# preethamam/AutomaticPanoramicImageStitching-AutoPanoStitch-MATLAB

Hardware: AMD Instinct MI355X
Metric: MPix/s end-to-end stitch (SIFT->blend), 64x4K images (higher is better)
Workload: dtype f32; 1 GPU

## Files before the change

### automaticpanoramicimagestitching-autopanostitch-matlab_amd/csrc/sift.hip

```cpp
#include <algorithm>
#include <cmath>
#include <cstring>
#include <vector>
#ifdef APS_DBG
#include <atomic>
#include <map>
#include <mutex>
#endif

#include "aps_internal.h"

#include <rocprim/rocprim.hpp>

namespace aps {

constexpr int kBorder = 5;
constexpr int kMaxInterp = 5;
constexpr int kOriBins = 36;
constexpr float kFix = 1048576.0f;

__device__ __forceinline__ long long to_fix(float v) { return (long long)(int)rintf(v * kFix); }
constexpr float kFltEps = 1.1920928955078125e-07f;

__device__ __forceinline__ float poly_exp2(float f) {
// ... 773 lines not shown
                                   unsigned int* __restrict__ flag) {
    const unsigned int i = blockIdx.x * blockDim.x + threadIdx.x;
    if (i >= n) return;
    flag[i] = (i == 0 || keys[i] != keys[i - 1]) ? 1u : 0u;
}
__global__ void compact_recs_kernel(const KpRec* __restrict__ recs, const unsigned int* __restrict__ idx,
                                    const unsigned int* __restrict__ flag, const unsigned int* __restrict__ pos,
                                    unsigned int n, KpRec* __restrict__ out) {
    const unsigned int i = blockIdx.x * blockDim.x + threadIdx.x;
    if (i >= n || !flag[i]) return;
    out[pos[i]] = recs[idx[i]];
}

struct PyrTable {
    OctaveDesc oct[16];
    int n_oct, nl;
    float sigma;
};

constexpr int kMW = 256;
constexpr int kMI = kMW - 8;
struct ExtremaPlan {
    int blk_ptr[17];
    int nstrip[16];
    int ch[16];
};

template <int nl>
__global__ __launch_bounds__(256) void extrema_march_kernel(const PyrTable* __restrict__ pt, ExtremaPlan plan, float thr,
                                                            unsigned long long* __restrict__ cells,
                                                            unsigned int* __restrict__ count, unsigned int cap) {
    constexpr int NG = nl + 3, ND = nl + 2, RING = 6, TW = kMW;
    __shared__ __attribute__((aligned(16))) float s_d[ND][RING * TW];
    constexpr int kLocalCap = 256;
    __shared__ unsigned long long s_cells[kLocalCap];
    __shared__ unsigned int s_n, s_base;
    int o = 0;
    while (o < 15 && (int)blockIdx.x >= plan.blk_ptr[o + 1]) ++o;
    const OctaveDesc& od = pt->oct[o];
    const int w = od.w, h = od.h;
    const int local = (int)blockIdx.x - plan.blk_ptr[o];
    const int strip = local % plan.nstrip[o], chunk = local / plan.nstrip[o];
    const int x0 = strip * kMI - 4, y0 = chunk * plan.ch[o], y1 = min(y0 + plan.ch[o], h);
    const int tid = threadIdx.x;
    if (tid == 0) s_n = 0u;
    const __attribute__((address_space(1))) float* G[NG];
#pragma unroll
    for (int p = 0; p < NG; ++p) G[p] = (const __attribute__((address_space(1))) float*)od.G[p];
    const int lx4 = tid & 63, lr = tid >> 6;
    const int gx = x0 + 4 * lx4;
    const bool vec = (w & 3) == 0 && gx >= 0 && gx + 3 < w;
    auto fetch = [&](int row, float4 g[NG]) __attribute__((always_inline)) {
        const size_t rowoff = (size_t)min(max(row, 0), h - 1) * w;
        if (vec) {
#pragma unroll
            for (int p = 0; p < NG; ++p) {
                typedef float f32x4g __attribute__((ext_vector_type(4)));
                const f32x4g v = *reinterpret_cast<const __attribute__((address_space(1))) f32x4g*>(G[p] + rowoff + gx);
                g[p] = make_float4(v.x, v.y, v.z, v.w);
            }
        } else {
            const size_t o0 = rowoff + min(max(gx, 0), w - 1), o1 = rowoff + min(max(gx + 1, 0), w - 1);
            const size_t o2 = rowoff + min(max(gx + 2, 0), w - 1), o3 = rowoff + min(max(gx + 3, 0), w - 1);
#pragma unroll
            for (int p = 0; p < NG; ++p) g[p] = make_float4(G[p][o0], G[p][o1], G[p][o2], G[p][o3]);
        }
    };
    auto park = [&](int row, const float4 g[NG]) __attribute__((always_inline)) {
        const int slot = (row - (y0 - 1)) % RING;
#pragma unroll
        for (int p = 0; p < ND; ++p)
            *reinterpret_cast<float4*>(&s_d[p][slot * TW + 4 * lx4]) =
                make_float4(g[p + 1].x - g[p].x, g[p + 1].y - g[p].y, g[p + 1].z - g[p].z, g[p + 1].w - g[p].w);
    };
    float4 g[NG];
    if (lr < 2) {
        fetch(y0 - 1 + lr, g);
        park(y0 - 1 + lr, g);
    }
    fetch(y0 + 1 + lr, g);
    const int lx = tid, c = x0 + lx;
    const int lxc = min(max(lx, 1), kMW - 2);
    const bool col_ok = lx >= 4 && lx < kMW - 4 && c >= kBorder && c < w - kBorder;
    for (int ys = y0; ys < y1; ys += 4) {
        park(ys + 1 + lr, g);
        if (ys + 4 < y1) fetch(ys + 5 + lr, g);
        __syncthreads();
        const int base = (ys - y0) % RING;
        float wmax[3][4], wmin[3][4];
#pragma unroll
        for (int p = 0; p < ND; ++p) {
            float hmx[6], hmn[6];
#pragma unroll
            for (int rr = 0; rr < 6; ++rr) {
                int slot = base + rr;
                slot = slot >= RING ? slot - RING : slot;
                const float* row = &s_d[p][slot * TW + lxc - 1];
                hmx[rr] = fmaxf(fmaxf(row[0], row[1]), row[2]);
                hmn[rr] = fminf(fminf(row[0], row[1]), row[2]);
            }
#pragma unroll
            for (int k = 0; k < 4; ++k) {
                wmax[p % 3][k] = fmaxf(fmaxf(hmx[k], hmx[k + 1]), hmx[k + 2]);
                wmin[p % 3][k] = fminf(fminf(hmn[k], hmn[k + 1]), hmn[k + 2]);
            }
            if (p < 2) continue;
            const int layer = p - 1;
#pragma unroll
            for (int k = 0; k < 4; ++k) {
                const int r = ys + k;
                if (!col_ok || r >= y1 || r < kBorder || r >= h - kBorder) continue;
                int slot = base + k + 1;
                slot = slot >= RING ? slot - RING : slot;
                const float val = s_d[layer][slot * TW + lx];
                if (!(fabsf(val) > thr)) continue;
                const float mx = fmaxf(fmaxf(wmax[0][k], wmax[1][k]), wmax[2][k]);
                const float mn = fminf(fminf(wmin[0][k], wmin[1][k]), wmin[2][k]);
                const bool is_max = val > 0 && val >= mx, is_min = val < 0 && val <= mn;
                if (!(is_max || is_min)) continue;
                const unsigned long long cell = ((unsigned long long)o << 40) | ((unsigned long long)layer << 32) |
                                                ((unsigned long long)r << 16) | (unsigned long long)c;
                const unsigned int loc = atomicAdd(&s_n, 1u);
                if (loc < (unsigned)kLocalCap) {
                    s_cells[loc] = cell;
                } else {
                    const unsigned int slot2 = atomicAdd(count, 1u);
                    if (slot2 < cap) cells[slot2] = cell;
                }
            }
        }
        __syncthreads();
    }
    const unsigned int n_loc = min(s_n, (unsigned)kLocalCap);
    if (n_loc == 0u) return;
    if (tid == 0) s_base = atomicAdd(count, n_loc);
    __syncthreads();
    for (unsigned int e = tid; e < n_loc; e += 256) {
        const unsigned int slot = s_base + e;
        if (slot < cap) cells[slot] = s_cells[e];
    }
}

constexpr int kWS = 124;
constexpr int kWCells = 256;
struct ExtremaWavePlan {
    int job_ptr[17];
    int nstrip[16];
    int ch[16];
};

__device__ __forceinline__ float dpp_from_lower_lane(float v) {
    return __int_as_float(__builtin_amdgcn_update_dpp(__float_as_int(v), __float_as_int(v), 0x138, 0xf, 0xf, false));
}
__device__ __forceinline__ float dpp_from_upper_lane(float v) {
    return __int_as_float(__builtin_amdgcn_update_dpp(__float_as_int(v), __float_as_int(v), 0x130, 0xf, 0xf, false));
}

template <int nl>
__global__ __launch_bounds__(256) void extrema_wave_kernel(const PyrTable* __restrict__ pt, ExtremaWavePlan plan, float thr,
                                                           unsigned long long* __restrict__ cells,
                                                           unsigned int* __restrict__ count, unsigned int cap) {
    constexpr int NG = nl + 3, ND = nl + 2;
    __shared__ unsigned long long s_cells[4][kWCells];
    const int lane = threadIdx.x & 63;
    const int wave = __builtin_amdgcn_readfirstlane(threadIdx.x >> 6);
    const int job = (int)blockIdx.x * 4 + wave;
    if (job >= plan.job_ptr[16]) return;
    int o = 0;
    while (o < 15 && job >= plan.job_ptr[o + 1]) ++o;
    const OctaveDesc& od = pt->oct[o];
    const int w = od.w, h = od.h;
    const int local = job - plan.job_ptr[o];
    const int strip = local % plan.nstrip[o], chunk = local / plan.nstrip[o];
    const int x0 = strip * kWS - 2, y0 = chunk * plan.ch[o], y1 = min(y0 + plan.ch[o], h);
    const int rc0 = max(y0, kBorder), rc1 = min(y1, h - kBorder);
    if (rc0 >= rc1) return;
    const __attribute__((address_space(1))) float* G[NG];
#pragma unroll
    for (int p = 0; p < NG; ++p) G[p] = (const __attribute__((address_space(1))) float*)od.G[p];
    const int c0 = x0 + 2 * lane;
    const int cb = min(max(c0, 0), w - 2);
    const bool own = lane >= 1 && lane <= 62;
    const bool ok0 = own && c0 >= kBorder && c0 < w - kBorder, ok1 = own && c0 + 1 >= kBorder && c0 + 1 < w - kBorder;
    typedef float f32x2g __attribute__((ext_vector_type(2)));
    f32x2g q[3][NG];
    auto fetch = [&](auto S, int row) __attribute__((always_inline)) {
        constexpr int sl = decltype(S)::value;
        const size_t off = (size_t)min(row, h - 1) * w + cb;
#pragma unroll
        for (int p = 0; p < NG; ++p) q[sl][p] = *reinterpret_cast<const __attribute__((address_space(1))) f32x2g*>(G[p] + off);
    };
    float hm[3][ND][2], hn[3][ND][2];
    float dc[3][nl][2];
    auto reduce_row = [&](auto S) __attribute__((always_inline)) {
        constexpr int sl = decltype(S)::value;
#pragma unroll
        for (int p = 0; p < ND; ++p) {
            const float d0 = q[sl][p + 1].x - q[sl][p].x, d1 = q[sl][p + 1].y - q[sl][p].y;
            const float lf = dpp_from_lower_lane(d1), rt = dpp_from_upper_lane(d0);
            hm[sl][p][0] = fmaxf(fmaxf(lf, d0), d1);
            hm[sl][p][1] = fmaxf(fmaxf(d0, d1), rt);
            hn[sl][p][0] = fminf(fminf(lf, d0), d1);
            hn[sl][p][1] = fminf(fminf(d0, d1), rt);
            if (p >= 1 && p <= nl) {
                dc[sl][p - 1][0] = d0;
                dc[sl][p - 1][1] = d1;
            }
        }
    };
    int qn = 0;
    auto emit = [&](bool pass, int layer, int r, int c) __attribute__((always_inline)) {
        const unsigned long long m = __ballot(pass);
        if (m == 0ull) return;
        if (pass) {
            const unsigned long long cell = ((unsigned long long)o << 40) | ((unsigned long long)layer << 32) |
                                            ((unsigned long long)r << 16) | (unsigned long long)c;
            const int at = qn + __popcll(m & ((1ull << lane) - 1ull));
            if (at < kWCells) {
                s_cells[wave][at] = cell;
            } else {
                const unsigned int slot2 = atomicAdd(count, 1u);
                if (slot2 < cap) cells[slot2] = cell;
            }
        }
        qn += __popcll(m);
    };
    auto test_row = [&](auto SA, auto SB, auto SC, int r) __attribute__((always_inline)) {
        constexpr int a = decltype(SA)::value, b = decltype(SB)::value, c = decltype(SC)::value;
        float wmax[3][2], wmin[3][2];
#pragma unroll
        for (int p = 0; p < ND; ++p) {
#pragma unroll
            for (int k = 0; k < 2; ++k) {
                wmax[p % 3][k] = fmaxf(fmaxf(hm[a][p][k], hm[b][p][k]), hm[c][p][k]);
                wmin[p % 3][k] = fminf(fminf(hn[a][p][k], hn[b][p][k]), hn[c][p][k]);
            }
            if (p < 2) continue;
            const int layer = p - 1;
#pragma unroll
            for (int k = 0; k < 2; ++k) {
                const float val = dc[b][layer - 1][k];
                const float mx = fmaxf(fmaxf(wmax[0][k], wmax[1][k]), wmax[2][k]);
                const float mn = fminf(fminf(wmin[0][k], wmin[1][k]), wmin[2][k]);
                const bool pass = (k ? ok1 : ok0) && fabsf(val) > thr && ((val > 0 && val >= mx) || (val < 0 && val <= mn));
                emit(pass, layer, r, c0 + k);
            }
        }
    };
    using I0 = std::integral_constant<int, 0>;
    using I1 = std::integral_constant<int, 1>;
    using I2 = std::integral_constant<int, 2>;
    fetch(I0{}, rc0 - 1);
    fetch(I1{}, rc0);
    fetch(I2{}, rc0 + 1);
    reduce_row(I0{});
    fetch(I0{}, rc0 + 2);
    reduce_row(I1{});
    fetch(I1{}, rc0 + 3);
    for (int r = rc0; r < rc1; r += 3) {
        reduce_row(I2{});
        fetch(I2{}, r + 4);
        test_row(I0{}, I1{}, I2{}, r);
        if (r + 1 >= rc1) break;
        reduce_row(I0{});
        fetch(I0{}, r + 5);
        test_row(I1{}, I2{}, I0{}, r + 1);
        if (r + 2 >= rc1) break;
        reduce_row(I1{});
        fetch(I1{}, r + 6);
        test_row(I2{}, I0{}, I1{}, r + 2);
    }
    if (qn == 0) return;
    const int n_loc = min(qn, kWCells);
    unsigned int base = 0;
    if (lane == 0) base = atomicAdd(count, (unsigned int)n_loc);
    base = __builtin_amdgcn_readfirstlane(base);
    __builtin_amdgcn_wave_barrier();
    for (int e = lane; e < n_loc; e += 64) {
        const unsigned int slot = base + e;
        if (slot < cap) cells[slot] = s_cells[wave][e];
    }
}

__global__ void refine_kernel(const PyrTable* __restrict__ pt, const unsigned long long* __restrict__ cells,
                              const unsigned int* __restrict__ n_cells, unsigned int cells_cap, float contr_thr,
                              float edge_thr, KpRec* __restrict__ recs, unsigned int* __restrict__ count,
                              unsigned int cap) {
    const unsigned int i = blockIdx.x * blockDim.x + threadIdx.x;
    const unsigned int n = min(*n_cells, cells_cap);
    if (i >= n) return;
    const unsigned long long key = cells[i];
    const int o = (int)(key >> 40), layer = (int)((key >> 32) & 0xff), r = (int)((key >> 16) & 0xffff),
              c = (int)(key & 0xffff);
    KpRec kp;
    if (!adjust_extremum(pt->oct[o], pt->nl, o, layer, r, c, contr_thr, edge_thr, kp)) return;
    const unsigned int slot = atomicAdd(count, 1u);
    if (slot < cap) recs[slot] = kp;
}

__device__ __forceinline__ float kp_scale(float sigma, int layer, float xi, int nl) {
    return sigma * my_exp2(((float)layer + xi) / (float)nl);
}

__global__ __launch_bounds__(256) void orient_kernel(const PyrTable* __restrict__ pt,
                                                     const KpRec* __restrict__ kps, unsigned int n,
                                                     unsigned int* __restrict__ ori_count,
                                                     float* __restrict__ ori_angle ,
                                                     unsigned char* __restrict__ ori_bin ) {
    __shared__ unsigned long long s_hist[4][kOriBins];
    __shared__ float s_h[4][kOriBins + 4];
    const int wv = threadIdx.x >> 6, lane = threadIdx.x & 63;
    const unsigned int ki = blockIdx.x * 4 + wv;
    const bool active = ki < n;
    if (lane < kOriBins) s_hist[wv][lane] = 0ull;
    __syncthreads();
    int o = 0, layer = 1, r0 = 0, c0 = 0;
    float xi = 0;
    if (active) {
        const KpRec kp = kps[ki];
        o = (int)(kp.key >> 40);
        layer = (int)((kp.key >> 32) & 0xff);
        r0 = (int)((kp.key >> 16) & 0xffff);
        c0 = (int)(kp.key & 0xffff);
        xi = kp.xi;
    }
    const OctaveDesc& od = pt->oct[o];
    const __attribute__((address_space(1))) float* g = (const __attribute__((address_space(1))) float*)od.G[layer];
    const int w = od.w, h = od.h;
    const float scl = kp_scale(pt->sigma, layer, xi, pt->nl);
    const int radius = (int)rintf(4.5f * scl);
    const float sig = 1.5f * scl;
    const float expf_scale = -1.0f / (2.0f * sig * sig);
    const int side = 2 * radius + 1;
    if (active) {
        for (int s = lane; s < side * side; s += 64) {
            const int i = s / side - radius, j = s % side - radius;
            const int y = r0 + i, x = c0 + j;
            if (y <= 0 || y >= h - 1 || x <= 0 || x >= w - 1) continue;
            const int ctr = y * w + x;
            const float dx = g[ctr + 1] - g[ctr - 1];
            const float dy = g[ctr - w] - g[ctr + w];
            const float wgt = my_exp((float)(i * i + j * j) * expf_scale);
            const float ori = fast_atan2_deg(dy, dx);
            const float mag = sqrtf(dx * dx + dy * dy);
            int bin = (int)rintf(((float)kOriBins / 360.0f) * ori);
            if (bin >= kOriBins) bin -= kOriBins;
            if (bin < 0) bin += kOriBins;
            const long long q = to_fix(wgt * mag);
            atomicAdd(&s_hist[wv][bin], (unsigned long long)q);
        }
    }
    __syncthreads();
    if (lane < kOriBins) s_h[wv][lane + 2] = (float)(long long)s_hist[wv][lane] * (1.0f / kFix);
    __syncthreads();
    if (lane < 2) {
        s_h[wv][lane] = s_h[wv][kOriBins + lane];
        s_h[wv][kOriBins + 2 + lane] = s_h[wv][2 + lane];
    }
    __syncthreads();
    float hv = 0.f;
    if (lane < kOriBins)
        hv = (s_h[wv][lane] + s_h[wv][lane + 4]) * (1.0f / 16.0f) + (s_h[wv][lane + 1] + s_h[wv][lane + 3]) * (4.0f / 16.0f) +
             s_h[wv][lane + 2] * (6.0f / 16.0f);
    __syncthreads();
    if (lane < kOriBins) s_h[wv][lane] = hv;
    __syncthreads();
    if (active) {
        float omax = lane < kOriBins ? s_h[wv][lane] : -INFINITY;
#pragma unroll
        for (int off = 32; off > 0; off >>= 1) omax = fmaxf(omax, __shfl_xor(omax, off));
        const float thr = omax * 0.8f;
        bool peak = false;
        float angle = 0.f;
        if (lane < kOriBins) {
            const int j = lane;
            const int l = j > 0 ? j - 1 : kOriBins - 1, r2 = j < kOriBins - 1 ? j + 1 : 0;
            const float hj = s_h[wv][j], hl = s_h[wv][l], hr = s_h[wv][r2];
            if (hj > hl && hj > hr && hj >= thr) {
                peak = true;
                float bin = (float)j + 0.5f * (hl - hr) / (hl - 2.0f * hj + hr);
                bin = bin < 0 ? (float)kOriBins + bin : (bin >= (float)kOriBins ? bin - (float)kOriBins : bin);
                angle = 360.0f - (360.0f / (float)kOriBins) * bin;
                if (fabsf(angle - 360.0f) < kFltEps) angle = 0.0f;
            }
        }
        const unsigned long long pm = __ballot(peak);
        if (peak) {
            const unsigned int cnt = (unsigned int)__popcll(pm & ((1ull << lane) - 1ull));
            ori_angle[(size_t)ki * kOriBins + cnt] = angle;
            ori_bin[(size_t)ki * kOriBins + cnt] = (unsigned char)lane;
        }
        if (lane == 0) ori_count[ki] = (unsigned int)__popcll(pm);
    }
}

struct OrientedKp {
    unsigned int kp;
    float angle;
};

__global__ void expand_oriented_kernel(const unsigned int* __restrict__ ori_count,
                                       const unsigned int* __restrict__ ori_pos,
                                       const float* __restrict__ ori_angle, unsigned int n,
                                       OrientedKp* __restrict__ out) {
    const unsigned int i = blockIdx.x * blockDim.x + threadIdx.x;
    if (i >= n) return;
    const unsigned int c = ori_count[i], p = ori_pos[i];
    for (unsigned int e = 0; e < c; ++e) {
        out[p + e].kp = i;
        out[p + e].angle = ori_angle[(size_t)i * kOriBins + e];
    }
}

constexpr int kD = 4, kN = 8, kHistLen = (kD + 2) * (kD + 2) * (kN + 2);
constexpr int kDescQueue = 512;

__global__ __launch_bounds__(256) void descr_kernel(const PyrTable* __restrict__ pt,
                                                    const KpRec* __restrict__ kps,
                                                    const OrientedKp* __restrict__ oks, unsigned int n_out,
                                                    float* __restrict__ desc, int desc_layout, int64_t ldd,
                                                    double* __restrict__ loc, int64_t ldl,
                                                    float* __restrict__ aux, int plain_sweep) {
    __shared__ unsigned long long s_hist[4][kHistLen];
    __shared__ __attribute__((aligned(16))) float s_raw[4][128];
    __shared__ int s_queue[4][kDescQueue];
    const int wv = threadIdx.x >> 6, lane = threadIdx.x & 63;
    const unsigned int oi = blockIdx.x * 4 + wv;
    const bool active = oi < n_out;
    for (int e = lane; e < kHistLen; e += 64) s_hist[wv][e] = 0ull;
    __syncthreads();
    int o = 0, layer = 1, r0 = 0, c0 = 0;
    float xc = 0, xr = 0, xi = 0, contr = 0, kangle = 0;
    if (active) {
        const OrientedKp ok = oks[oi];
        const KpRec kp = kps[ok.kp];
        o = (int)(kp.key >> 40);
        layer = (int)((kp.key >> 32) & 0xff);
        r0 = (int)((kp.key >> 16) & 0xffff);
        c0 = (int)(kp.key & 0xffff);
        xc = kp.xc;
        xr = kp.xr;
        xi = kp.xi;
        contr = kp.contr;
        kangle = ok.angle;
    }
    const OctaveDesc& od = pt->oct[o];
    const __attribute__((address_space(1))) float* g = (const __attribute__((address_space(1))) float*)od.G[layer];
    const int w = od.w, h = od.h;
    const float scl = kp_scale(pt->sigma, layer, xi, pt->nl);
    float ori = 360.0f - kangle;
    if (fabsf(ori - 360.0f) < kFltEps) ori = 0.0f;
    const float ptx = (float)c0 + xc, pty = (float)r0 + xr;
    const int px = (int)rintf(ptx), py = (int)rintf(pty);
    float sin_t, cos_t;
    sincos_deg(ori, sin_t, cos_t);
    const float bins_per_deg = (float)kN / 360.0f;
    const float exp_scale = -1.0f / ((float)(kD * kD) * 0.5f);
    const float hist_width = 3.0f * scl;
    int radius = (int)rintf(hist_width * 1.4142135623730951f * (float)(kD + 1) * 0.5f);
    const int diag = (int)sqrt((double)w * w + (double)h * h);
    if (radius > diag) radius = diag;
    cos_t = cos_t / hist_width;
    sin_t = sin_t / hist_width;
    const int side = 2 * radius + 1;
    (void)side;
    auto accumulate = [&](int i, int j) __attribute__((always_inline)) {
        const float c_rot = (float)j * cos_t - (float)i * sin_t;
        const float r_rot = (float)j * sin_t + (float)i * cos_t;
        float rbin = r_rot + (float)(kD / 2) - 0.5f;
        float cbin = c_rot + (float)(kD / 2) - 0.5f;
        const int r = py + i, c = px + j;
        const int ctr = r * w + c;
        const float dx = g[ctr + 1] - g[ctr - 1];
        const float dy = g[ctr - w] - g[ctr + w];
        const float wgt = my_exp((c_rot * c_rot + r_rot * r_rot) * exp_scale);
        const float o_deg = fast_atan2_deg(dy, dx);
        const float mag = sqrtf(dx * dx + dy * dy) * wgt;
        float obin = (o_deg - ori) * bins_per_deg;
        const int rr0 = (int)floorf(rbin), cc0 = (int)floorf(cbin);
        int o0 = (int)floorf(obin);
        rbin -= (float)rr0;
        cbin -= (float)cc0;
        obin -= (float)o0;
        if (o0 < 0) o0 += kN;
        if (o0 >= kN) o0 -= kN;
        const float v_r1 = mag * rbin, v_r0 = mag - v_r1;
        const float v_rc11 = v_r1 * cbin, v_rc10 = v_r1 - v_rc11;
        const float v_rc01 = v_r0 * cbin, v_rc00 = v_r0 - v_rc01;
        const float v111 = v_rc11 * obin, v110 = v_rc11 - v111;
        const float v101 = v_rc10 * obin, v100 = v_rc10 - v101;
        const float v011 = v_rc01 * obin, v010 = v_rc01 - v011;
        const float v001 = v_rc00 * obin, v000 = v_rc00 - v001;
        const int idx = ((rr0 + 1) * (kD + 2) + cc0 + 1) * (kN + 2) + o0;
        unsigned long long* hb = &s_hist[wv][idx];
#define ADDQ(off, v) atomicAdd(hb + (off), (unsigned long long)to_fix(v))
        ADDQ(0, v000);
        ADDQ(1, v001);
        ADDQ(kN + 2, v010);
        ADDQ(kN + 3, v011);
        ADDQ((kD + 2) * (kN + 2), v100);
        ADDQ((kD + 2) * (kN + 2) + 1, v101);
        ADDQ((kD + 3) * (kN + 2), v110);
        ADDQ((kD + 3) * (kN + 2) + 1, v111);
#undef ADDQ
    };
    if (active) {
        int* q = s_queue[wv];
        int qn = 0;
        auto flush = [&]() __attribute__((always_inline)) {
            const int rounds = (qn + 63) >> 6;
            __builtin_amdgcn_wave_barrier();
            const int e0 = lane * rounds;
            int pk = q[min(e0, kDescQueue - 1)];
            for (int r = 0; r < rounds; ++r) {
                const int e = e0 + r;
                const int pk_next = q[min(e + 1, kDescQueue - 1)];
                if (e < qn) accumulate(pk >> 16, (int)(short)(pk & 0xffff));
                pk = pk_next;
            }
            __builtin_amdgcn_wave_barrier();
            qn = 0;
        };
        auto passes = [&](int i, int j) __attribute__((always_inline)) {
            const float c_rot = (float)j * cos_t - (float)i * sin_t;
            const float r_rot = (float)j * sin_t + (float)i * cos_t;
            const float rbin = r_rot + (float)(kD / 2) - 0.5f;
            const float cbin = c_rot + (float)(kD / 2) - 0.5f;
            const int r = py + i, c = px + j;
            return j >= -radius && j <= radius && rbin > -1 && rbin < kD && cbin > -1 && cbin < kD && r > 0 && r < h - 1 && c > 0 && c < w - 1;
        };
        bool plain = plain_sweep != 0 || radius > 63 || fabsf(sin_t) < 1e-4f || fabsf(cos_t) < 1e-4f;
        int jl_[2] = {0, 0}, len_[2] = {0, 0};
        if (!plain) {
            bool bad = false;
#pragma unroll
            for (int half = 0; half < 2; ++half) {
                const int i = -radius + lane + 64 * half;
                const bool row_ok = i <= radius && py + i > 0 && py + i < h - 1;
                const float fi = (float)i;
                float lo = fmaxf(-(float)radius, (float)(1 - px)), hi = fminf((float)radius, (float)(w - 2 - px));
                auto clip = [&](float a, float lo_v, float hi_v) __attribute__((always_inline)) {
                    const float p0 = lo_v / a, p1 = hi_v / a;
                    lo = fmaxf(lo, fminf(p0, p1));
                    hi = fminf(hi, fmaxf(p0, p1));
                };
                clip(sin_t, -2.5f - fi * cos_t, 2.5f - fi * cos_t);
                clip(cos_t, -2.5f + fi * sin_t, 2.5f + fi * sin_t);
                const int gl = (int)ceilf(lo), gh = (int)floorf(hi);
                int jl = 0x7fffffff, jh = -0x7fffffff;
#pragma unroll
                for (int dlt = 2; dlt >= -2; --dlt)
                    if (passes(i, gl + dlt)) jl = gl + dlt;
#pragma unroll
                for (int dlt = -2; dlt <= 2; ++dlt)
                    if (passes(i, gh + dlt)) jh = gh + dlt;
                const bool none = jl > jh;
                bool good;
                if (none)
                    good = gl > gh;
                else
                    good = !passes(i, jl - 1) && !passes(i, jh + 1) && passes(i, (jl + jh) / 2) && jl >= gl - 2 && jh <= gh + 2;
                bad = bad || (row_ok && !good);
                jl_[half] = jl;
                len_[half] = (row_ok && !none) ? jh - jl + 1 : 0;
            }
            plain = __any(bad) != 0;
        }
        if (!plain) {
#pragma unroll
            for (int half = 0; half < 2; ++half) {
                unsigned long long rows_m = __ballot(len_[half] > 0);
                while (rows_m) {
                    const int l = __ffsll((long long)rows_m) - 1;
                    rows_m &= rows_m - 1ull;
                    const int rj = __builtin_amdgcn_readlane(jl_[half], l), rn = __builtin_amdgcn_readlane(len_[half], l);
                    const int ri = -radius + l + 64 * half;
                    for (int t0 = 0; t0 < rn; t0 += 64) {
                        const int cnt = min(64, rn - t0);
                        if (lane < cnt) q[qn + lane] = (ri << 16) | ((rj + t0 + lane) & 0xffff);
                        qn += cnt;
                        if (qn > kDescQueue - 64) flush();
                    }
                }
            }
        } else {
            for (int i = -radius; i <= radius; ++i) {
                for (int j0 = -radius; j0 <= radius; j0 += 64) {
                    const int j = j0 + lane;
                    const bool pass = passes(i, j);
                    const unsigned long long m = __ballot(pass);
                    if (m == 0ull) continue;
                    if (pass) q[qn + __popcll(m & ((1ull << lane) - 1ull))] = (i << 16) | (j & 0xffff);
                    qn += __popcll(m);
                    if (qn > kDescQueue - 64) flush();
                }
            }
        }
        if (qn > 0) flush();
    }
    __syncthreads();
#pragma unroll
    for (int half = 0; half < 2; ++half) {
        const int e = lane + 64 * half;
        const int k = e & 7, ij = e >> 3, i = ij >> 2, j = ij & 3;
        const int idx = ((i + 1) * (kD + 2) + (j + 1)) * (kN + 2);
        long long v = (long long)s_hist[wv][idx + k];
        if (k < 2) v += (long long)s_hist[wv][idx + kN + k];
        s_raw[wv][e] = (float)v * (1.0f / kFix);
    }
    __syncthreads();
    if (!active) return;
    auto sumsq = [&]() __attribute__((always_inline)) {
        float a = 0;
#pragma unroll 4
        for (int k4 = 0; k4 < 32; ++k4) {
            const float4 v = *reinterpret_cast<const float4*>(&s_raw[wv][4 * k4]);
            a = fmaf(v.x, v.x, a);
            a = fmaf(v.y, v.y, a);
            a = fmaf(v.z, v.z, a);
            a = fmaf(v.w, v.w, a);
        }
        return a;
    };
    float nrm2 = sumsq();
    const float thr = sqrtf(nrm2) * 0.2f;
    float clip[2];
#pragma unroll
    for (int half = 0; half < 2; ++half) {
        const float v0 = s_raw[wv][lane + 64 * half];
        clip[half] = v0 < thr ? v0 : thr;
    }
    __builtin_amdgcn_wave_barrier();
    s_raw[wv][lane] = clip[0];
    s_raw[wv][lane + 64] = clip[1];
    __builtin_amdgcn_wave_barrier();
    nrm2 = sumsq();
    const float sn = sqrtf(nrm2);
    const float scale = 512.0f / (sn > kFltEps ? sn : kFltEps);
    float qv[2];
#pragma unroll
    for (int half = 0; half < 2; ++half) {
        float v = rintf(clip[half] * scale);
        qv[half] = v < 0 ? 0 : (v > 255 ? 255 : v);
    }
    __builtin_amdgcn_wave_barrier();
    s_raw[wv][lane] = qv[0];
    s_raw[wv][lane + 64] = qv[1];
    __builtin_amdgcn_wave_barrier();
    const float qq = sumsq();
    const float inv = sqrtf(qq);
#pragma unroll
    for (int half = 0; half < 2; ++half) {
        const int e = lane + 64 * half;
        const float outv = inv > 0 ? qv[half] / inv : 0.0f;
        if (desc_layout == APS_ROWMAJOR)
            desc[(size_t)oi * ldd + e] = outv;
        else
            desc[(size_t)e * ldd + oi] = outv;
    }
    if (lane == 0) {
        const float s = ldexpf(1.0f, o) * 0.5f;
        loc[oi] = (double)(ptx * s) + 1.0;
        loc[ldl + oi] = (double)(pty * s) + 1.0;
        if (aux) {
            aux[(size_t)oi * 4 + 0] = scl * s * 2.0f;
            aux[(size_t)oi * 4 + 1] = kangle;
            aux[(size_t)oi * 4 + 2] = contr;
            aux[(size_t)oi * 4 + 3] = (float)(o + 256 * layer);
        }
    }
}

static GaussK make_gauss(double sigma) {
    GaussK g;
    int n = (int)std::lrint(sigma * 8.0 + 1.0) | 1;
    if (n > 63) n = 63;
    const double s2 = -0.5 / (sigma * sigma);
    double sum = 0;
    for (int i = 0; i < n; ++i) {
        const double x = i - (n - 1) * 0.5;
        g.k[i] = (float)std::exp(s2 * x * x);
        sum += g.k[i];
    }
    sum = 1.0 / sum;
    for (int i = 0; i < n; ++i) g.k[i] = (float)(g.k[i] * sum);
    g.n = n;
    return g;
}

static bool launch_blur(const float* in, int h, int w, double sigma, float* out, Ws<float>& scratch, float* dec = nullptr,
                        int dh = 0, int dw = 0) {
    const GaussK gk = make_gauss(sigma);
    const int r = gk.n / 2;
    Prof prof("sift_blur");
    const dim3 grid(cdiv(w, kTW), cdiv(h, kTH));
    static const bool march = std::getenv("APS_BLUR_MARCH") != nullptr;
    if (march && r >= 1 && r <= 12 && h >= 64 && w >= kSW) {
        const int strips = cdiv(w, kSW);
        int ch = (int)(((long long)h * strips + 1023) / 1024);
        ch = std::max(4 * kRS, (ch + kRS - 1) / kRS * kRS);
        const dim3 mg(strips, cdiv(h, ch));
        switch (r) {
#define APS_BLUR_CASE(R) \
    case R:              \
        blur_march_kernel<R><<<mg, 256, 0, stream()>>>(in, h, w, gk, out, dec, dh, dw, ch); \
        break;
            APS_BLUR_CASE(1)
            APS_BLUR_CASE(2)
            APS_BLUR_CASE(3)
            APS_BLUR_CASE(4)
            APS_BLUR_CASE(5)
            APS_BLUR_CASE(6)
            APS_BLUR_CASE(7)
            APS_BLUR_CASE(8)
            APS_BLUR_CASE(9)
            APS_BLUR_CASE(10)
            APS_BLUR_CASE(11)
            APS_BLUR_CASE(12)
#undef APS_BLUR_CASE
        }
        check_launch("blur_march_kernel");
        return dec != nullptr;
    }
    switch (r) {
#define APS_BLUR_CASE(R) \
    case R:              \
        blur_kernel<R><<<grid, 256, 0, stream()>>>(in, h, w, gk, out, dec, dh, dw); \
        break;
        APS_BLUR_CASE(1)
        APS_BLUR_CASE(2)
        APS_BLUR_CASE(3)
        APS_BLUR_CASE(4)
        APS_BLUR_CASE(5)
        APS_BLUR_CASE(6)
        APS_BLUR_CASE(7)
        APS_BLUR_CASE(8)
        APS_BLUR_CASE(9)
        APS_BLUR_CASE(10)
        APS_BLUR_CASE(11)
        APS_BLUR_CASE(12)
#undef APS_BLUR_CASE
        default: {
            if (scratch.n < (size_t)h * w) scratch.alloc((size_t)h * w);
            blur_row_generic<<<dim3(cdiv(w, 256), h), 256, 0, stream()>>>(in, h, w, gk, scratch);
            blur_col_generic<<<dim3(cdiv(w, 256), h), 256, 0, stream()>>>(scratch, h, w, gk, out);
            dec = nullptr;
        }
    }
    check_launch("blur_kernel");
    return dec != nullptr;
}

static bool launch_base_blur(const uint8_t* img, int sh, int sw, int c, int layout, double sigma, float* out, Ws<uint8_t>& gray) {
    static const bool off = [] {
        const char* e = std::getenv("APS_SIFT_NO_BASE_FUSE");
        return e && e[0] == '1';
    }();
    if (off) return false;
    const GaussK gk = make_gauss(sigma);
    const int r = (gk.n - 1) / 2;
    if (r < 3 || r > 8) return false;
    const dim3 grid(cdiv(2 * sw, kTW), cdiv(2 * sh, kTH));
    Prof prof("sift_blur");
    gray.alloc((size_t)sh * sw);
    gray_u8_kernel<<<dim3(cdiv(cdiv(sw, 4), 256), sh), 256, 0, stream()>>>(img, sh, sw, c, layout, gray);
    switch (r) {
#define APS_BLUR_CASE(R) \
    case R:              \
        blur_base_kernel<R><<<grid, 256, 0, stream()>>>(gray, sh, sw, gk, out); \
        break;
        APS_BLUR_CASE(3)
        APS_BLUR_CASE(4)
        APS_BLUR_CASE(5)
        APS_BLUR_CASE(6)
        APS_BLUR_CASE(7)
        APS_BLUR_CASE(8)
#undef APS_BLUR_CASE
        default: return false;
    }
    check_launch("blur_base_kernel");
    return true;
}

static int num_octaves(int H, int W) {
    const int mn = std::min(2 * W, 2 * H);
    return (int)std::lrint(std::log((double)mn) / std::log(2.0) - 2.0) + 1;
}


#ifdef APS_DBG
namespace dbg {
enum { kPyrChanged, kExtReplays, kExtDiff, kRefReplays, kRefDiff, kOriReplays, kOriDiff, kOriWords, kDesReplays, kDesDiff, kDesWords, kCalls, kNStat };
static std::atomic<long long> g_stat[kNStat];
static std::mutex g_mu;
static std::map<const void*, unsigned long long> g_pyr;
__global__ void cks_kernel(const unsigned int* __restrict__ p, size_t n_rec, int wpr, int positional, unsigned long long* __restrict__ out) {
    const size_t i = blockIdx.x * (size_t)blockDim.x + threadIdx.x;
    unsigned long long h = 0;
    if (i < n_rec) {
        h = 0x9E3779B97F4A7C15ull;
        for (int k = 0; k < wpr; ++k) {
            h ^= p[i * wpr + k];
            h *= 0x100000001B3ull;
            h ^= h >> 29;
        }
        if (positional) h *= (2ull * i + 1ull);
    }
#pragma unroll
    for (int off = 32; off > 0; off >>= 1) h += __shfl_xor(h, off);
    if ((threadIdx.x & 63) == 0 && h) atomicAdd(out, h);
}
__global__ void diff_kernel(const unsigned int* __restrict__ a, const unsigned int* __restrict__ b, size_t n, unsigned long long* __restrict__ out) {
    const size_t i = blockIdx.x * (size_t)blockDim.x + threadIdx.x;
    const unsigned long long m = __ballot(i < n && a[i] != b[i]);
    if ((threadIdx.x & 63) == 0 && m) atomicAdd(out, (unsigned long long)__popcll(m));
}
static unsigned long long cks(const void* p, size_t n_rec, int wpr, int positional, unsigned long long* d_slot) {
    APS_HIP(hipMemsetAsync(d_slot, 0, 8, stream()));
    if (n_rec) cks_kernel<<<cdiv(n_rec, 256), 256, 0, stream()>>>((const unsigned int*)p, n_rec, wpr, positional, d_slot);
    unsigned long long h = 0;
    APS_HIP(hipMemcpyAsync(&h, d_slot, 8, hipMemcpyDeviceToHost, stream()));
    APS_HIP(hipStreamSynchronize(stream()));
    return h;
}
static unsigned long long diff(const void* a, const void* b, size_t n_words, unsigned long long* d_slot) {
    APS_HIP(hipMemsetAsync(d_slot, 0, 8, stream()));
    if (n_words) diff_kernel<<<cdiv(n_words, 256), 256, 0, stream()>>>((const unsigned int*)a, (const unsigned int*)b, n_words, d_slot);
    unsigned long long h = 0;
    APS_HIP(hipMemcpyAsync(&h, d_slot, 8, hipMemcpyDeviceToHost, stream()));
    APS_HIP(hipStreamSynchronize(stream()));
    return h;
}
}
#endif
}

using namespace aps;

extern "C" {

int aps_sift_extract(const uint8_t* img, int height, int width, int channels, int img_layout,
                     const aps_sift_params* params, float* desc, int desc_layout, int64_t ldd,
                     double* loc, int64_t ldl, float* aux, int64_t cap, int64_t* count) {
    return guarded([&] {
        APS_REQUIRE(img && params && count, APS_E_ARG, "NULL argument");
        APS_REQUIRE(height > 0 && width > 0, APS_E_DIM, "empty image");
        APS_REQUIRE(channels == 1 || channels == 3, APS_E_DIM, "channels must be 1 or 3");
        APS_REQUIRE(img_layout == APS_IMG_U8_HWC || img_layout == APS_IMG_U8_MATLAB, APS_E_TYPE, "unknown image layout");
        APS_REQUIRE(desc_layout == APS_ROWMAJOR || desc_layout == APS_COLMAJOR, APS_E_TYPE, "unknown descriptor layout");
        APS_REQUIRE(params->n_layers >= 1 && params->n_layers <= 5, APS_E_ARG, "NumLayersInOctave must be in 1..5");
        APS_REQUIRE(params->sigma > 0.5, APS_E_ARG, "Sigma must exceed the assumed camera blur 0.5");
        APS_REQUIRE(params->contrast_threshold >= 0 && params->edge_threshold >= 1, APS_E_ARG, "bad thresholds");
        APS_REQUIRE(cap >= 0, APS_E_ARG, "negative capacity");
        APS_REQUIRE(2 * (int64_t)height < 65536 && 2 * (int64_t)width < 65536, APS_E_DIM, "image side must be < 32768");
        ctx();
        *count = 0;
        const int nl = params->n_layers;
        const int H = height, W = width;
        In<uint8_t> dimg(img, (size_t)H * W * channels);
        Ws<float> up, scratch;
        Ws<uint8_t> gray8;
        const int n_oct = std::min(num_octaves(H, W), 16);
        if (n_oct <= 0) return;
        std::vector<Ws<float>> G((size_t)n_oct * (nl + 3));
        PyrTable table;
        std::memset(&table, 0, sizeof table);
        table.n_oct = n_oct;
        table.nl = nl;
        table.sigma = (float)params->sigma;
        double sig[16];
        sig[0] = params->sigma;
        const double kf = std::pow(2.0, 1.0 / nl);
        for (int i = 1; i < nl + 3; ++i) {
            const double sp = std::pow(kf, (double)(i - 1)) * params->sigma, st = sp * kf;
            sig[i] = std::sqrt(st * st - sp * sp);
        }
        int ow = 2 * W, oh = 2 * H;
        bool base_written = false;
        for (int o = 0; o < n_oct; ++o) {
            if (o > 0) {
                ow = std::max(1, ow / 2);
                oh = std::max(1, oh / 2);
            }
            OctaveDesc& od = table.oct[o];
            od.w = ow;
            od.h = oh;
            const size_t px = (size_t)ow * oh;
            for (int i = 0; i < nl + 3; ++i)
                if (!(i == 0 && base_written)) G[o * (nl + 3) + i].alloc(px);
            if (o == 0) {
                double sd = params->sigma * params->sigma - 4.0 * 0.5 * 0.5;
                if (sd < 0.01) sd = 0.01;
                if (!launch_base_blur(dimg, H, W, channels, img_layout, std::sqrt(sd), G[0], gray8)) {
                    up.alloc((size_t)4 * H * W);
                    gray_up_kernel<<<dim3(cdiv(2 * W, kGUW), cdiv(2 * H, kGUH)), 256, 0, stream()>>>(dimg, H, W, channels, img_layout, up);
                    check_launch("gray_up_kernel");
                    launch_blur(up, oh, ow, std::sqrt(sd), G[0], scratch);
                }
            } else if (!base_written) {
                const OctaveDesc& pd = table.oct[o - 1];
                decimate_kernel<<<dim3(cdiv(ow, 256), oh), 256, 0, stream()>>>(G[(o - 1) * (nl + 3) + nl], pd.h, pd.w,
                                                                            oh, ow, G[o * (nl + 3)]);
                check_launch("decimate_kernel");
            }
            base_written = false;
            for (int i = 1; i < nl + 3; ++i) {
                if (i == nl && o + 1 < n_oct) {
                    const int nw = std::max(1, ow / 2), nh = std::max(1, oh / 2);
                    G[(o + 1) * (nl + 3)].alloc((size_t)nw * nh);
                    base_written = launch_blur(G[o * (nl + 3) + i - 1], oh, ow, sig[i], G[o * (nl + 3) + i], scratch,
                                               G[(o + 1) * (nl + 3)], nh, nw);
// ... 311 lines not shown
```

Before: 3224 MPix/s.

## Privatize SIFT orientation/descriptor histograms into per-lane copies and drop padding bins

Result: faster. 3265 MPix/s, median of 6 (+1.3%).

```diff
diff --git a/automaticpanoramicimagestitching-autopanostitch-matlab_amd/csrc/sift.hip b/automaticpanoramicimagestitching-autopanostitch-matlab_amd/csrc/sift.hip
--- a/automaticpanoramicimagestitching-autopanostitch-matlab_amd/csrc/sift.hip
+++ b/automaticpanoramicimagestitching-autopanostitch-matlab_amd/csrc/sift.hip
@@ -1099,17 +1099,19 @@
     return sigma * my_exp2(((float)layer + xi) / (float)nl);
 }
 
+constexpr int kOriCopies = 4;
+
 __global__ __launch_bounds__(256) void orient_kernel(const PyrTable* __restrict__ pt,
                                                      const KpRec* __restrict__ kps, unsigned int n,
                                                      unsigned int* __restrict__ ori_count,
                                                      float* __restrict__ ori_angle ,
                                                      unsigned char* __restrict__ ori_bin ) {
-    __shared__ unsigned long long s_hist[4][kOriBins];
+    __shared__ unsigned long long s_hist[4][kOriCopies][kOriBins];
     __shared__ float s_h[4][kOriBins + 4];
     const int wv = threadIdx.x >> 6, lane = threadIdx.x & 63;
     const unsigned int ki = blockIdx.x * 4 + wv;
     const bool active = ki < n;
-    if (lane < kOriBins) s_hist[wv][lane] = 0ull;
+    for (int e = lane; e < kOriCopies * kOriBins; e += 64) (&s_hist[wv][0][0])[e] = 0ull;
     __syncthreads();
     int o = 0, layer = 1, r0 = 0, c0 = 0;
     float xi = 0;
@@ -1130,8 +1132,14 @@
     const float expf_scale = -1.0f / (2.0f * sig * sig);
     const int side = 2 * radius + 1;
     if (active) {
-        for (int s = lane; s < side * side; s += 64) {
-            const int i = s / side - radius, j = s % side - radius;
+        const int di = 64 / side, dj = 64 % side;
+        int i = lane / side - radius, j = lane % side - radius;
+        unsigned long long* hb = s_hist[wv][lane & (kOriCopies - 1)];
+        for (int s = lane; s < side * side; s += 64, i += di, j += dj) {
+            if (j > radius) {
+                j -= side;
+                ++i;
+            }
             const int y = r0 + i, x = c0 + j;
             if (y <= 0 || y >= h - 1 || x <= 0 || x >= w - 1) continue;
             const int ctr = y * w + x;
@@ -1144,11 +1152,16 @@
             if (bin >= kOriBins) bin -= kOriBins;
             if (bin < 0) bin += kOriBins;
             const long long q = to_fix(wgt * mag);
-            atomicAdd(&s_hist[wv][bin], (unsigned long long)q);
+            atomicAdd(hb + bin, (unsigned long long)q);
         }
     }
     __syncthreads();
-    if (lane < kOriBins) s_h[wv][lane + 2] = (float)(long long)s_hist[wv][lane] * (1.0f / kFix);
+    if (lane < kOriBins) {
+        unsigned long long v = 0;
+#pragma unroll
+        for (int cp = 0; cp < kOriCopies; ++cp) v += s_hist[wv][cp][lane];
+        s_h[wv][lane + 2] = (float)(long long)v * (1.0f / kFix);
+    }
     __syncthreads();
     if (lane < 2) {
         s_h[wv][lane] = s_h[wv][kOriBins + lane];
@@ -1209,7 +1222,8 @@
     }
 }
 
-constexpr int kD = 4, kN = 8, kHistLen = (kD + 2) * (kD + 2) * (kN + 2);
+constexpr int kD = 4, kN = 8, kHistLen = kD * kD * kN;
+constexpr int kDescCopies = 2;
 constexpr int kDescQueue = 512;
 
 __global__ __launch_bounds__(256) void descr_kernel(const PyrTable* __restrict__ pt,
@@ -1218,13 +1232,13 @@
                                                     float* __restrict__ desc, int desc_layout, int64_t ldd,
                                                     double* __restrict__ loc, int64_t ldl,
                                                     float* __restrict__ aux, int plain_sweep) {
-    __shared__ unsigned long long s_hist[4][kHistLen];
+    __shared__ unsigned long long s_hist[4][kDescCopies][kHistLen];
     __shared__ __attribute__((aligned(16))) float s_raw[4][128];
     __shared__ int s_queue[4][kDescQueue];
     const int wv = threadIdx.x >> 6, lane = threadIdx.x & 63;
     const unsigned int oi = blockIdx.x * 4 + wv;
     const bool active = oi < n_out;
-    for (int e = lane; e < kHistLen; e += 64) s_hist[wv][e] = 0ull;
+    for (int e = lane; e < kDescCopies * kHistLen; e += 64) (&s_hist[wv][0][0])[e] = 0ull;
     __syncthreads();
     int o = 0, layer = 1, r0 = 0, c0 = 0;
     float xc = 0, xr = 0, xi = 0, contr = 0, kangle = 0;
@@ -1288,17 +1302,27 @@
         const float v101 = v_rc10 * obin, v100 = v_rc10 - v101;
         const float v011 = v_rc01 * obin, v010 = v_rc01 - v011;
         const float v001 = v_rc00 * obin, v000 = v_rc00 - v001;
-        const int idx = ((rr0 + 1) * (kD + 2) + cc0 + 1) * (kN + 2) + o0;
-        unsigned long long* hb = &s_hist[wv][idx];
-#define ADDQ(off, v) atomicAdd(hb + (off), (unsigned long long)to_fix(v))
-        ADDQ(0, v000);
-        ADDQ(1, v001);
-        ADDQ(kN + 2, v010);
-        ADDQ(kN + 3, v011);
-        ADDQ((kD + 2) * (kN + 2), v100);
-        ADDQ((kD + 2) * (kN + 2) + 1, v101);
-        ADDQ((kD + 3) * (kN + 2), v110);
-        ADDQ((kD + 3) * (kN + 2) + 1, v111);
+        const int o1 = o0 == kN - 1 ? 0 : o0 + 1;
+        const bool r0ok = rr0 >= 0, r1ok = rr0 < kD - 1, c0ok = cc0 >= 0, c1ok = cc0 < kD - 1;
+        unsigned long long* hb = s_hist[wv][lane & (kDescCopies - 1)];
+        const int base = (rr0 * kD + cc0) * kN;
+#define ADDQ(off, v) atomicAdd(hb + base + (off), (unsigned long long)to_fix(v))
+        if (r0ok && c0ok) {
+            ADDQ(o0, v000);
+            ADDQ(o1, v001);
+        }
+        if (r0ok && c1ok) {
+            ADDQ(kN + o0, v010);
+            ADDQ(kN + o1, v011);
+        }
+        if (r1ok && c0ok) {
+            ADDQ(kD * kN + o0, v100);
+            ADDQ(kD * kN + o1, v101);
+        }
+        if (r1ok && c1ok) {
+            ADDQ((kD + 1) * kN + o0, v110);
+            ADDQ((kD + 1) * kN + o1, v111);
+        }
 #undef ADDQ
     };
     if (active) {
@@ -1399,11 +1423,10 @@
 #pragma unroll
     for (int half = 0; half < 2; ++half) {
         const int e = lane + 64 * half;
-        const int k = e & 7, ij = e >> 3, i = ij >> 2, j = ij & 3;
-        const int idx = ((i + 1) * (kD + 2) + (j + 1)) * (kN + 2);
-        long long v = (long long)s_hist[wv][idx + k];
-        if (k < 2) v += (long long)s_hist[wv][idx + kN + k];
-        s_raw[wv][e] = (float)v * (1.0f / kFix);
+        unsigned long long v = 0;
+#pragma unroll
+        for (int cp = 0; cp < kDescCopies; ++cp) v += s_hist[wv][cp][e];
+        s_raw[wv][e] = (float)(long long)v * (1.0f / kFix);
     }
     __syncthreads();
     if (!active) return;
```
